# gabry1998/Self-Supervised-Anomaly-Detection

Hardware: AMD Instinct MI355X
Metric: train images/sec + anomaly-maps/sec, ResNet-18 256x256 bs256 (higher is better)
Workload: dtype f32; 1 GPU; ResNet-18 256x256 bs256 self-sup train + anomaly map, 1xMI355X, synthetic images (BASELINE configs[1]); images_per_gpu=256, global_batch=256, patches_per_image=841, bank_rows=588, parallelism=dp1 (256 images), train_step_launch=hipGraph segments, train_graph_segments=1

## Files before the change

### self-supervised-anomaly-detection_amd/csrc/stem.hip

```cpp
#include "common.h"
#include <type_traits>

namespace {

constexpr int STEM_MAX_GRID = 4096;


constexpr int TOH = 8, TOW = 32;
constexpr int TIH = TOH * 2 + 5;
constexpr int TIW = 72;
constexpr int KSTEPS = 7 * 4 * 3;
constexpr int IN_TILE = TIH * TIW * 3;
constexpr int W_TILE = KSTEPS * 2 * 64;

struct StemParams {
    const float* img;
    const float* wk;
    const float* scale;
    const float* shift;
    float* out;
    int B, H, W, pd, ps, Hv, Wv, Ho, Wo, relu;
    int prow, pcol;
    int ph, pw;
    int tiles_y, tiles_x;
    int64_t total_tiles;
    int64_t Nsamp;
    int hwnc;
    double* stats;
};

__global__ __launch_bounds__(256, 2) void stem_conv7x7_kernel(StemParams p) {
    extern __shared__ __attribute__((aligned(16))) float lds[];
    float* wl = lds;
    float* tin = lds + W_TILE;
    const int tid = threadIdx.x, lane = tid & 63, wave = tid >> 6;
    const int r = lane & 31, h = lane >> 5;

    for (int i = tid; i < W_TILE / 4; i += 256) ((f32x4*)wl)[i] = ((const f32x4*)p.wk)[i];

    float sc[2], sh[2];
#pragma unroll
    for (int j = 0; j < 2; ++j) {
        sc[j] = p.scale ? p.scale[j * 32 + r] : 1.f;
        sh[j] = p.shift ? p.shift[j * 32 + r] : 0.f;
    }

    double st0[2] = {0.0, 0.0}, st1[2] = {0.0, 0.0};
    const int tiles_per_sample = p.tiles_y * p.tiles_x;
    const bool direct = p.ph == p.Hv && p.pw == p.Wv;
    const int64_t plane = (int64_t)p.H * p.W;
    constexpr int NIN = (TIH * TIW + 255) / 256;
    float pv[NIN][3];
    auto fetch_tile = [&](int64_t t) {
        const int64_t n = t / tiles_per_sample;
        const int tt = (int)(t - n * tiles_per_sample);
        const int ty0 = (tt / p.tiles_x) * TOH, tx0 = (tt % p.tiles_x) * TOW;
        const int P = p.prow * p.pcol;
        const int b = (int)(n / P);
        const int pi = (int)(n - (int64_t)b * P);
        const int y0 = (pi / p.pcol) * p.ps, x0 = (pi % p.pcol) * p.ps;
        const float* src = p.img + (int64_t)b * 3 * plane;
#pragma unroll
        for (int q = 0; q < NIN; ++q) {
            const int i = tid + 256 * q;
            const int iy = i / TIW, ix = i - iy * TIW;
            const int vy = 2 * ty0 - 3 + iy, vx = 2 * tx0 - 3 + ix;
            float v0 = 0.f, v1 = 0.f, v2 = 0.f;
            if (i < TIH * TIW && (unsigned)vy < (unsigned)p.Hv && (unsigned)vx < (unsigned)p.Wv) {
                const int sy = y0 + (direct ? vy : (vy * p.ph) / p.Hv), sx = x0 + (direct ? vx : (vx * p.pw) / p.Wv);
                const float* s = src + (int64_t)sy * p.W + sx;
                v0 = s[0]; v1 = s[plane]; v2 = s[2 * plane];
            }
            pv[q][0] = v0; pv[q][1] = v1; pv[q][2] = v2;
        }
    };
    if ((int64_t)blockIdx.x < p.total_tiles) fetch_tile(blockIdx.x);
    for (int64_t t = blockIdx.x; t < p.total_tiles; t += gridDim.x) {
        const int64_t n = t / tiles_per_sample;
        const int tt = (int)(t - n * tiles_per_sample);
        const int ty0 = (tt / p.tiles_x) * TOH, tx0 = (tt % p.tiles_x) * TOW;

        __syncthreads();
#pragma unroll
        for (int q = 0; q < NIN; ++q) {
            const int i = tid + 256 * q;
            if (i < TIH * TIW) {
                float* d = tin + i * 3;
                d[0] = pv[q][0]; d[1] = pv[q][1]; d[2] = pv[q][2];
            }
        }
        __syncthreads();
        if (t + gridDim.x < p.total_tiles) fetch_tile(t + gridDim.x);

        f32x16 acc[2][2];
#pragma unroll
        for (int i = 0; i < 2; ++i)
#pragma unroll
            for (int j = 0; j < 2; ++j)
#pragma unroll
                for (int e = 0; e < 16; ++e) acc[i][j][e] = 0.f;
        const float* a0 = tin + ((2 * (2 * wave + 0)) * TIW + 2 * r + h) * 3;
        const float* a1 = tin + ((2 * (2 * wave + 1)) * TIW + 2 * r + h) * 3;
        const float* bw = wl + h * 64 + r;
#pragma unroll
        for (int ky = 0; ky < 7; ++ky)
#pragma unroll
            for (int q = 0; q < 4; ++q)
#pragma unroll
                for (int c = 0; c < 3; ++c) {
                    const int ko = (ky * TIW + 2 * q) * 3 + c;
                    const int kb = ((ky * 4 + q) * 3 + c) * 128;
                    float x0v = a0[ko], x1v = a1[ko];
                    float w0 = bw[kb], w1 = bw[kb + 32];
                    acc[0][0] = mfma32(x0v, w0, acc[0][0]);
                    acc[0][1] = mfma32(x0v, w1, acc[0][1]);
                    acc[1][0] = mfma32(x1v, w0, acc[1][0]);
                    acc[1][1] = mfma32(x1v, w1, acc[1][1]);
                }

        if (tx0 + 32 <= p.Wo) {
            const int64_t pst = p.hwnc ? p.Nsamp * 256 : 256;
            const unsigned lane_off = (unsigned)((int64_t)(4 * h) * pst + r * 4);
            typedef float f32x2v __attribute__((ext_vector_type(2)));
            auto rows = [&](auto stats_tag) __attribute__((always_inline)) {
                constexpr bool ST = decltype(stats_tag)::value;
                const float lowb = p.relu ? 0.f : -__builtin_huge_valf();
#pragma unroll
                for (int i = 0; i < 2; ++i) {
                    const int oy = ty0 + 2 * wave + i;
                    if (oy >= p.Ho) continue;
                    const int64_t pix0 = p.hwnc ? ((int64_t)oy * p.Wo + tx0) * p.Nsamp + n : (n * p.Ho + oy) * p.Wo + tx0;
                    char* const ob = (char*)(p.out + pix0 * 64);
#pragma unroll
                    for (int j = 0; j < 2; ++j) {
                        f32x2v ps = {0.f, 0.f}, pq = {0.f, 0.f};
#pragma unroll
                        for (int e = 0; e < 16; e += 2) {
                            f32x2v v = {acc[i][j][e], acc[i][j][e + 1]};
                            if (ST) {
                                ps += v;
                                pq = v * v + pq;
                            } else {
                                v = v * f32x2v{sc[j], sc[j]} + f32x2v{sh[j], sh[j]};
                                v[0] = fmaxf(v[0], lowb); v[1] = fmaxf(v[1], lowb);
                            }
#pragma unroll
                            for (int k = 0; k < 2; ++k)
                                *(float*)(ob + (int64_t)(((e + k) & 3) + 8 * ((e + k) >> 2)) * pst + j * 128 + lane_off) = v[k];
                        }
                        if (ST) { st0[j] += (double)ps[0] + (double)ps[1]; st1[j] += (double)pq[0] + (double)pq[1]; }
                    }
                }
            };
            if (p.stats && !p.scale && !p.shift && !p.relu) { rows(std::true_type()); continue; }
            if (!p.stats) { rows(std::false_type()); continue; }
        }
#pragma unroll
        for (int i = 0; i < 2; ++i) {
            const int oy = ty0 + 2 * wave + i;
            if (oy >= p.Ho) continue;
#pragma unroll
            for (int j = 0; j < 2; ++j) {
                float fs = 0.f, fq = 0.f;
#pragma unroll
                for (int e = 0; e < 16; ++e) {
                    int ox = tx0 + (e & 3) + 8 * (e >> 2) + 4 * h;
                    if (ox < p.Wo) {
                        if (p.stats) { fs += acc[i][j][e]; fq += acc[i][j][e] * acc[i][j][e]; }
                        float v = acc[i][j][e] * sc[j] + sh[j];
                        if (p.relu) v = fmaxf(v, 0.f);
                        const int64_t pix = p.hwnc ? ((int64_t)oy * p.Wo + ox) * p.Nsamp + n : (n * p.Ho + oy) * p.Wo + ox;
                        p.out[pix * 64 + j * 32 + r] = v;
                    }
                }
                if (p.stats) { st0[j] += (double)fs; st1[j] += (double)fq; }
            }
        }
    }
    if (p.stats) {
        __syncthreads();
        double* S = (double*)lds;
#pragma unroll
        for (int j = 0; j < 2; ++j) {
            st0[j] += __shfl_xor(st0[j], 32);
            st1[j] += __shfl_xor(st1[j], 32);
            if (h == 0) {
                S[(wave * 2 + 0) * 64 + j * 32 + r] = st0[j];
                S[(wave * 2 + 1) * 64 + j * 32 + r] = st1[j];
            }
        }
        __syncthreads();
        if (tid < 128) {
            const int which = tid >> 6, cc = tid & 63;
            p.stats[((int64_t)blockIdx.x * 2 + which) * 64 + cc] =
                ((S[(0 * 2 + which) * 64 + cc] + S[(1 * 2 + which) * 64 + cc]) + S[(2 * 2 + which) * 64 + cc]) + S[(3 * 2 + which) * 64 + cc];
        }
    }
}

constexpr int SP_SW = 40, SP_SH = 36;
constexpr int SP_SRC = SP_SH * SP_SW * 3;
constexpr int SP_WF = 24 * 2 * 64;
constexpr int SP_CB = 9 * 32 * 32;

struct StemPatchParams {
    const float* img;
    const float* wf;
    const float* scale;
    const float* shift;
    float* out;
    int B, H, W, ps, prow, pcol, hwnc;
    int skip_lo, skip_hi;
    int64_t Nsamp;
};

__global__ __launch_bounds__(256, 2) void stem_patch_fused_kernel(StemPatchParams p) {
    extern __shared__ __attribute__((aligned(16))) float lds[];
    float* wl = lds;
    float* src = lds + SP_WF;
    float* cb = src + SP_SRC;
    const int tid = threadIdx.x, lane = tid & 63, wave = tid >> 6;
    const int r = lane & 31, h = lane >> 5;
    for (int i = tid; i < SP_WF / 4; i += 256) ((f32x4*)wl)[i] = ((const f32x4*)p.wf)[i];
    const int P = p.prow * p.pcol;
    const int64_t plane = (int64_t)p.H * p.W;

    constexpr int NSRC = (SP_SH * SP_SW + 255) / 256;
    float pv[NSRC][3];
    auto fetch_patch = [&](int64_t n) {
        const int b = (int)(n / P);
        const int pi = (int)(n - (int64_t)b * P);
        const int y0 = (pi / p.pcol) * p.ps, x0 = (pi % p.pcol) * p.ps;
        const float* im = p.img + (int64_t)b * 3 * plane;
#pragma unroll
        for (int q = 0; q < NSRC; ++q) {
            const int i = tid + 256 * q;
            const int ty = i / SP_SW, tx = i - ty * SP_SW;
            const int sy = ty - 2, sx = tx - 2;
            float v0 = 0.f, v1 = 0.f, v2 = 0.f;
            if (i < SP_SH * SP_SW && (unsigned)sy < 32u && (unsigned)sx < 32u) {
                const float* s = im + (int64_t)(y0 + sy) * p.W + x0 + sx;
                v0 = s[0]; v1 = s[plane]; v2 = s[2 * plane];
            }
            pv[q][0] = v0; pv[q][1] = v1; pv[q][2] = v2;
        }
    };
    if ((int64_t)blockIdx.x < p.Nsamp) fetch_patch(blockIdx.x);
    for (int64_t n = blockIdx.x; n < p.Nsamp; n += gridDim.x) {
        __syncthreads();
#pragma unroll
        for (int q = 0; q < NSRC; ++q) {
            const int i = tid + 256 * q;
            if (i < SP_SH * SP_SW) {
                float* d = src + i * 3;
                d[0] = pv[q][0]; d[1] = pv[q][1]; d[2] = pv[q][2];
            }
        }
        if (n + gridDim.x < p.Nsamp) fetch_patch(n + gridDim.x);
        for (int pass = 0; pass < 2; ++pass) {
            const float sc = p.scale ? p.scale[pass * 32 + r] : 1.f;
            const float sh = p.shift ? p.shift[pass * 32 + r] : 0.f;
            for (int i = tid; i < 32 * 32; i += 256) cb[i] = 0.f;
            __syncthreads();
            for (int t = 0; t < 4; ++t) {
                f32x16 acc0, acc1;
#pragma unroll
                for (int e = 0; e < 16; ++e) { acc0[e] = 0.f; acc1[e] = 0.f; }
                const int oy = 8 * t + 2 * wave;
                const float* a0 = src + ((oy + 0) * SP_SW + r + h) * 3;
                const float* a1 = src + ((oy + 1) * SP_SW + r + h) * 3;
                const float* bw = wl + h * 64 + pass * 32 + r;
// ... 39 lines not shown
                ((f32x4*)cb)[tid] = ((const f32x4*)(cb + 8 * 32 * 32))[tid];
                __syncthreads();
            }
        }
    }
}

constexpr int SB_CB = 7 * 32 * 32;

__global__ __launch_bounds__(256, 2) void stem_patch_border_kernel(StemPatchParams p) {
    extern __shared__ __attribute__((aligned(16))) float lds[];
    float* wl = lds;
    float* src = lds + SP_WF;
    float* cb = src + SP_SRC;
    const int tid = threadIdx.x, lane = tid & 63, wave = tid >> 6;
    const int r = lane & 31, h = lane >> 5;
    for (int i = tid; i < SP_WF / 4; i += 256) ((f32x4*)wl)[i] = ((const f32x4*)p.wf)[i];
    const int P = p.prow * p.pcol;
    const int64_t plane = (int64_t)p.H * p.W;
    constexpr int NSRC = (SP_SH * SP_SW + 255) / 256;
    float pv[NSRC][3];
    auto fetch_patch = [&](int64_t n) {
        const int b = (int)(n / P);
        const int pi = (int)(n - (int64_t)b * P);
        const int y0 = (pi / p.pcol) * p.ps, x0 = (pi % p.pcol) * p.ps;
        const float* im = p.img + (int64_t)b * 3 * plane;
#pragma unroll
        for (int q = 0; q < NSRC; ++q) {
            const int i = tid + 256 * q;
            const int ty = i / SP_SW, tx = i - ty * SP_SW;
            const int sy = ty - 2, sx = tx - 2;
            float v0 = 0.f, v1 = 0.f, v2 = 0.f;
            if (i < SP_SH * SP_SW && (unsigned)sy < 32u && (unsigned)sx < 32u) {
                const float* s = im + (int64_t)(y0 + sy) * p.W + x0 + sx;
                v0 = s[0]; v1 = s[plane]; v2 = s[2 * plane];
            }
            pv[q][0] = v0; pv[q][1] = v1; pv[q][2] = v2;
        }
    };
    auto row_of = [](int t) { return t < 4 ? t : 25 + t; };
    const int ta0 = 2 * wave, ta1 = 2 * wave + 1 < 7 ? 2 * wave + 1 : 2 * wave;
    const float* pa0 = src + (row_of(ta0) * SP_SW + r + h) * 3;
    const float* pa1 = src + (row_of(ta1) * SP_SW + r + h) * 3;
    const float *pb0, *pb1;
    {
        int q0 = (2 * wave) * 32 + r, q1 = (2 * wave + 1) * 32 + r;
        q0 = q0 < 189 ? q0 : 188; q1 = q1 < 189 ? q1 : 188;
        const int c0 = q0 % 7, c1 = q1 % 7;
        pb0 = src + ((3 + q0 / 7) * SP_SW + (c0 < 4 ? c0 : 25 + c0) + h) * 3;
        pb1 = src + ((3 + q1 / 7) * SP_SW + (c1 < 4 ? c1 : 25 + c1) + h) * 3;
    }
    auto two_tiles = [&](const float* a0, const float* a1, int pass, f32x16& acc0, f32x16& acc1) {
#pragma unroll
        for (int e = 0; e < 16; ++e) { acc0[e] = 0.f; acc1[e] = 0.f; }
        const float* bw = wl + h * 64 + pass * 32 + r;
#pragma unroll
        for (int a = 0; a < 4; ++a)
#pragma unroll
            for (int q = 0; q < 2; ++q)
#pragma unroll
                for (int c = 0; c < 3; ++c) {
                    const int ko = (a * SP_SW + 2 * q) * 3 + c;
                    const float w = bw[((a * 2 + q) * 3 + c) * 128];
                    acc0 = mfma32(a0[ko], w, acc0);
                    acc1 = mfma32(a1[ko], w, acc1);
                }
    };
    if ((int64_t)blockIdx.x < p.Nsamp) fetch_patch(blockIdx.x);
    for (int64_t n = blockIdx.x; n < p.Nsamp; n += gridDim.x) {
        __syncthreads();
#pragma unroll
        for (int q = 0; q < NSRC; ++q) {
            const int i = tid + 256 * q;
            if (i < SP_SH * SP_SW) {
                float* d = src + i * 3;
                d[0] = pv[q][0]; d[1] = pv[q][1]; d[2] = pv[q][2];
            }
        }
        if (n + gridDim.x < p.Nsamp) fetch_patch(n + gridDim.x);
        __syncthreads();
        for (int pass = 0; pass < 2; ++pass) {
            const float sc = p.scale ? p.scale[pass * 32 + r] : 1.f;
            const float sh = p.shift ? p.shift[pass * 32 + r] : 0.f;
            f32x16 acc0, acc1;
            two_tiles(pa0, pa1, pass, acc0, acc1);
#pragma unroll
            for (int e = 0; e < 16; ++e) {
                const int ox = (e & 3) + 8 * (e >> 2) + 4 * h;
                cb[((2 * wave) * 32 + ox) * 32 + r] = fmaxf(acc0[e] * sc + sh, 0.f);
                if (2 * wave + 1 < 7) cb[((2 * wave + 1) * 32 + ox) * 32 + r] = fmaxf(acc1[e] * sc + sh, 0.f);
            }
            __syncthreads();
            for (int item = tid; item < 3 * 16 * 8; item += 256) {
                const int c4 = item & 7, px = (item >> 3) & 15, pr = item >> 7;
                const int t_lo = pr == 0 ? 0 : pr == 1 ? 1 : 4, t_hi = pr == 0 ? 1 : pr == 1 ? 3 : 6;
                f32x4 m = {0.f, 0.f, 0.f, 0.f};
                for (int t = t_lo; t <= t_hi; ++t)
#pragma unroll
                    for (int dx = -1; dx < 2; ++dx) {
                        const int cx = 2 * px + dx;
                        if (cx < 0) continue;
                        const f32x4 v = *(const f32x4*)(cb + (t * 32 + cx) * 32 + c4 * 4);
                        m[0] = fmaxf(m[0], v[0]); m[1] = fmaxf(m[1], v[1]); m[2] = fmaxf(m[2], v[2]); m[3] = fmaxf(m[3], v[3]);
                    }
                const int py = pr < 2 ? pr : 15;
                *(f32x4*)(p.out + (((int64_t)py * 16 + px) * p.Nsamp + n) * 64 + pass * 32 + c4 * 4) = m;
            }
            __syncthreads();
            if (wave < 3) {
                two_tiles(pb0, pb1, pass, acc0, acc1);
#pragma unroll
                for (int e = 0; e < 16; ++e) {
                    const int i = (e & 3) + 8 * (e >> 2) + 4 * h;
                    const int q0 = (2 * wave) * 32 + i, q1 = q0 + 32;
                    if (q0 < 189) cb[q0 * 32 + r] = fmaxf(acc0[e] * sc + sh, 0.f);
                    if (q1 < 189) cb[q1 * 32 + r] = fmaxf(acc1[e] * sc + sh, 0.f);
                }
            }
            __syncthreads();
            for (int item = tid; item < 13 * 3 * 8; item += 256) {
                const int c4 = item & 7, k = item >> 3, pk = k % 3, py = 2 + k / 3;
                const int ci_lo = pk == 0 ? 0 : pk == 1 ? 1 : 4, ci_hi = pk == 0 ? 1 : pk == 1 ? 3 : 6;
                f32x4 m = {0.f, 0.f, 0.f, 0.f};
#pragma unroll
                for (int dy = -1; dy < 2; ++dy)
                    for (int ci = ci_lo; ci <= ci_hi; ++ci) {
                        const f32x4 v = *(const f32x4*)(cb + ((2 * py + dy - 3) * 7 + ci) * 32 + c4 * 4);
                        m[0] = fmaxf(m[0], v[0]); m[1] = fmaxf(m[1], v[1]); m[2] = fmaxf(m[2], v[2]); m[3] = fmaxf(m[3], v[3]);
                    }
                const int px = pk < 2 ? pk : 15;
                *(f32x4*)(p.out + (((int64_t)py * 16 + px) * p.Nsamp + n) * 64 + pass * 32 + c4 * 4) = m;
            }
            __syncthreads();
        }
    }
}

__global__ void pack_stem_weight_folded_kernel(const float* __restrict__ w, float* __restrict__ wf) {
    const int i = blockIdx.x * blockDim.x + threadIdx.x;
    if (i >= SP_WF) return;
    const int co = i & 63, hh = (i >> 6) & 1, s = i >> 7;
    const int c = s % 3, q = (s / 3) & 1, a = s / 6;
    const int b = 2 * q + hh;
    const int ky0 = a == 0 ? 0 : 2 * a - 1, ky1 = a == 0 ? 0 : 2 * a;
    const int kx0 = b == 0 ? 0 : 2 * b - 1, kx1 = b == 0 ? 0 : 2 * b;
    float acc = 0.f;
    for (int ky = ky0; ky <= ky1; ++ky)
        for (int kx = kx0; kx <= kx1; ++kx) acc += w[((co * 3 + c) * 7 + ky) * 7 + kx];
    wf[i] = acc;
}

__global__ void pack_stem_weight_kernel(const float* __restrict__ w, float* __restrict__ wk, int ohwi = 0) {
    int i = blockIdx.x * blockDim.x + threadIdx.x;
    if (i >= 168 * 64) return;
    int co = i & 63, kl = i >> 6;
    int hh = kl & 1, rest = kl >> 1;
    int c = rest % 3, q = (rest / 3) & 3, ky = rest / 12;
    int kx = 2 * q + hh;
    const int src = ohwi ? ((co * 7 + ky) * 7 + (kx < 7 ? kx : 0)) * 3 + c : ((co * 3 + c) * 7 + ky) * 7 + (kx < 7 ? kx : 0);
    const float v = w[src];
    wk[i] = kx < 7 ? v : 0.f;
}

struct PoolBN { const float* mean; const float* invstd; const float* gamma; const float* beta; };

template <typename T>
__global__ __launch_bounds__(256) void maxpool3x3s2_kernel(const T* __restrict__ in, T* __restrict__ out, uint8_t* __restrict__ idx,
                                    int64_t totalE, int H, int W, int CE, int Ho, int Wo, int64_t N, int hwnc, PoolBN bn,
                                    T* __restrict__ zwin = nullptr) {
    constexpr int E = Lane<T>::E;
    using V = typename Lane<T>::vec;
    int64_t i = (int64_t)blockIdx.x * blockDim.x + threadIdx.x;
    if (i >= totalE) return;
    int cq = (int)(i % CE);
    int64_t pix = i / CE;
    int ox, oy;
    int64_t n;
    if (hwnc) {
        n = pix % N;
        int64_t t = pix / N;
        ox = (int)(t % Wo);
        oy = (int)(t / Wo);
    } else {
        ox = (int)(pix % Wo);
        int64_t t = pix / Wo;
        oy = (int)(t % Ho);
        n = t / Ho;
    }
    V m = -INFINITY, zw = 0.f;
    int am[E];
#pragma unroll
    for (int k = 0; k < E; ++k) am[k] = 0;
    V mu = 0.f, is = 0.f, ga = 0.f, be = 0.f;
    if (bn.mean) {
        mu = ldpar<V>(bn.mean, cq); is = ldpar<V>(bn.invstd, cq);
        ga = ldpar<V>(bn.gamma, cq); be = ldpar<V>(bn.beta, cq);
    }
    V tap[9];
#pragma unroll
    for (int dy = 0; dy < 3; ++dy) {
#pragma unroll
        for (int dx = 0; dx < 3; ++dx) {
            const int y = oy * 2 - 1 + dy, x = ox * 2 - 1 + dx;
            const bool ok = (unsigned)y < (unsigned)H && (unsigned)x < (unsigned)W;
            const int yc = ok ? y : oy * 2, xc = ok ? x : ox * 2;
            const int64_t ip = hwnc ? ((int64_t)yc * W + xc) * N + n : (n * H + yc) * W + xc;
            tap[dy * 3 + dx] = ldv(in + E * (ip * CE + cq));
        }
    }
#pragma unroll
    for (int dy = 0; dy < 3; ++dy) {
        int y = oy * 2 - 1 + dy;
        if ((unsigned)y >= (unsigned)H) continue;
#pragma unroll
        for (int dx = 0; dx < 3; ++dx) {
            int x = ox * 2 - 1 + dx;
            if ((unsigned)x >= (unsigned)W) continue;
            V v = tap[dy * 3 + dx];
            const V raw = v;
            if (bn.mean) {
#pragma unroll
                for (int k = 0; k < E; ++k) v[k] = stored<T>(fmaxf((v[k] - mu[k]) * is[k] * ga[k] + be[k], 0.f));
            }
#pragma unroll
            for (int k = 0; k < E; ++k)
                if (v[k] > m[k]) { m[k] = v[k]; am[k] = dy * 3 + dx; zw[k] = raw[k]; }
        }
    }
    stv(out + E * i, m);
    if (zwin) stv(zwin + E * i, zw);
    if (idx) {
#pragma unroll
        for (int q = 0; q < E / 4; ++q)
            ((uint32_t*)idx)[i * (E / 4) + q] = (uint32_t)am[4 * q] | ((uint32_t)am[4 * q + 1] << 8) | ((uint32_t)am[4 * q + 2] << 16) |
                                                ((uint32_t)am[4 * q + 3] << 24);
    }
}

}

extern "C" int ssad_pack_stem_weight(const float* w_oihw, float* wk, void* stream) {
    SSAD_CHECK_ARG(w_oihw && wk, "null pointer");
    hipLaunchKernelGGL(pack_stem_weight_kernel, dim3((168 * 64 + 255) / 256), dim3(256), 0, (hipStream_t)stream, w_oihw, wk, 0);
    SSAD_CHECK_LAUNCH();
    return 0;
}

extern "C" int ssad_pack_stem_weight_ohwi(const float* w_ohwi, float* wk, void* stream) {
    SSAD_CHECK_ARG(w_ohwi && wk, "null pointer");
    hipLaunchKernelGGL(pack_stem_weight_kernel, dim3((168 * 64 + 255) / 256), dim3(256), 0, (hipStream_t)stream, w_ohwi, wk, 1);
    SSAD_CHECK_LAUNCH();
    return 0;
}

static int stem_fwd_impl(const float* img, int B, int H, int W, int patch_dim, int patch_stride, int Hv, int Wv,
                         const float* wk, const float* scale, const float* shift, int relu, int hwnc, float* out,
                         void* stream, double* stats, int* stat_rows) {
    SSAD_CHECK_ARG(img && wk && out, "null pointer");
    SSAD_CHECK_ARG(B > 0 && H > 0 && W > 0 && Hv > 0 && Wv > 0, "empty shape");
    StemParams p;
    p.img = img; p.wk = wk; p.scale = scale; p.shift = shift; p.out = out;
    p.B = B; p.H = H; p.W = W; p.pd = patch_dim; p.ps = patch_stride; p.Hv = Hv; p.Wv = Wv; p.relu = relu;
    if (patch_dim > 0) {
        SSAD_CHECK_ARG(patch_stride > 0 && patch_dim <= H && patch_dim <= W, "bad patch window");
        p.prow = (H - patch_dim) / patch_stride + 1;
        p.pcol = (W - patch_dim) / patch_stride + 1;
        p.ph = p.pw = patch_dim;
    } else {
        p.prow = p.pcol = 1; p.ph = H; p.pw = W; p.ps = 0;
    }
    p.Ho = (Hv - 1) / 2 + 1;
    p.Wo = (Wv - 1) / 2 + 1;
    p.tiles_y = (p.Ho + TOH - 1) / TOH;
    p.tiles_x = (p.Wo + TOW - 1) / TOW;
    p.Nsamp = (int64_t)B * p.prow * p.pcol;
    p.hwnc = hwnc;
    p.stats = stats;
    p.total_tiles = p.Nsamp * p.tiles_y * p.tiles_x;
    constexpr int lds_bytes = (W_TILE + IN_TILE) * 4;
    static bool attr_set = false;
    if (!attr_set) {
        SSAD_SET_DYN_LDS(stem_conv7x7_kernel, lds_bytes);
        attr_set = true;
    }
    int64_t grid = p.total_tiles < STEM_MAX_GRID ? p.total_tiles : STEM_MAX_GRID;
    hipLaunchKernelGGL(stem_conv7x7_kernel, dim3((unsigned)grid), dim3(256), lds_bytes, (hipStream_t)stream, p);
    SSAD_CHECK_LAUNCH();
    if (stat_rows) *stat_rows = (int)grid;
    return 0;
}

extern "C" int ssad_stem_fwd(const float* img, int B, int H, int W, int patch_dim, int patch_stride, int Hv, int Wv,
                             const float* wk, const float* scale, const float* shift, int relu, int hwnc, float* out,
                             void* stream) {
    return stem_fwd_impl(img, B, H, W, patch_dim, patch_stride, Hv, Wv, wk, scale, shift, relu, hwnc, out, stream, nullptr, nullptr);
}

extern "C" int ssad_stem_stats_rows(void) { return STEM_MAX_GRID; }

extern "C" int ssad_stem_fwd_stats(const float* img, int B, int H, int W, int Hv, int Wv, const float* wk, float* out, float eps,
                                   float momentum, float* mean, float* invstd, float* running_mean, float* running_var,
                                   double* workspace, void* stream) {
    SSAD_CHECK_ARG(mean && invstd && workspace, "null pointer");
    int rows = 0;
    const int rc = stem_fwd_impl(img, B, H, W, 0, 0, Hv, Wv, wk, nullptr, nullptr, 0, 0, out, stream, workspace, &rows);
    if (rc) return rc;
    const int Ho = (Hv - 1) / 2 + 1, Wo = (Wv - 1) / 2 + 1;
    return ssad_bn_finalize_partials(workspace, rows, (int64_t)B * Ho * Wo, 64, eps, momentum, mean, invstd, running_mean,
                                     running_var, stream);
}

extern "C" int ssad_pack_stem_weight_folded(const float* w_oihw, float* wf, void* stream) {
    SSAD_CHECK_ARG(w_oihw && wf, "null pointer");
    hipLaunchKernelGGL(pack_stem_weight_folded_kernel, dim3((SP_WF + 255) / 256), dim3(256), 0, (hipStream_t)stream, w_oihw, wf);
    SSAD_CHECK_LAUNCH();
    return 0;
}

extern "C" int ssad_stem_patch_pool_fwd_ring(const float* img, int B, int H, int W, int patch_stride, const float* wf,
                                             const float* scale, const float* shift, int hwnc, int skip_lo, int skip_hi, float* out,
                                             void* stream);
extern "C" int ssad_stem_patch_pool_fwd(const float* img, int B, int H, int W, int patch_stride, const float* wf,
                                        const float* scale, const float* shift, int hwnc, float* out, void* stream) {
    return ssad_stem_patch_pool_fwd_ring(img, B, H, W, patch_stride, wf, scale, shift, hwnc, 1, 0, out, stream);
}
extern "C" int ssad_stem_patch_pool_fwd_ring(const float* img, int B, int H, int W, int patch_stride, const float* wf,
                                             const float* scale, const float* shift, int hwnc, int skip_lo, int skip_hi, float* out,
                                             void* stream) {
    SSAD_CHECK_ARG(img && wf && out, "null pointer");
    SSAD_CHECK_ARG(skip_lo > skip_hi || (skip_lo >= 0 && skip_hi < 16), "skipped square outside the 16 x 16 map");
    SSAD_CHECK_ARG(B > 0 && H >= 32 && W >= 32 && patch_stride > 0, "bad shape (32x32 windows)");
    StemPatchParams p;
    p.img = img; p.wf = wf; p.scale = scale; p.shift = shift; p.out = out;
    p.B = B; p.H = H; p.W = W; p.ps = patch_stride; p.hwnc = hwnc; p.skip_lo = skip_lo; p.skip_hi = skip_hi;
    p.prow = (H - 32) / patch_stride + 1;
    p.pcol = (W - 32) / patch_stride + 1;
    p.Nsamp = (int64_t)B * p.prow * p.pcol;
    constexpr int lds_bytes = (SP_WF + SP_SRC + SP_CB) * 4;
    static bool attr_set = false;
    if (!attr_set) {
        SSAD_SET_DYN_LDS(stem_patch_fused_kernel, lds_bytes);
        attr_set = true;
    }
    const int64_t grid = p.Nsamp < 2048 ? p.Nsamp : 2048;
    hipLaunchKernelGGL(stem_patch_fused_kernel, dim3((unsigned)grid), dim3(256), lds_bytes, (hipStream_t)stream, p);
    SSAD_CHECK_LAUNCH();
    return 0;
}

extern "C" int ssad_stem_patch_border_fwd(const float* img, int B, int H, int W, int patch_stride, const float* wf, const float* scale,
                                          const float* shift, float* out, void* stream) {
    SSAD_CHECK_ARG(img && wf && out, "null pointer");
    SSAD_CHECK_ARG(B > 0 && H >= 32 && W >= 32 && patch_stride > 0, "bad shape (32x32 windows)");
    StemPatchParams p;
    p.img = img; p.wf = wf; p.scale = scale; p.shift = shift; p.out = out;
    p.B = B; p.H = H; p.W = W; p.ps = patch_stride; p.hwnc = 1; p.skip_lo = 1; p.skip_hi = 0;
    p.prow = (H - 32) / patch_stride + 1;
    p.pcol = (W - 32) / patch_stride + 1;
    p.Nsamp = (int64_t)B * p.prow * p.pcol;
    constexpr int lds_bytes = (SP_WF + SP_SRC + SB_CB) * 4;
    static bool attr_set = false;
    if (!attr_set) {
        SSAD_SET_DYN_LDS(stem_patch_border_kernel, lds_bytes);
        attr_set = true;
    }
    const int64_t grid = p.Nsamp < 2048 ? p.Nsamp : 2048;
    hipLaunchKernelGGL(stem_patch_border_kernel, dim3((unsigned)grid), dim3(256), lds_bytes, (hipStream_t)stream, p);
    SSAD_CHECK_LAUNCH();
    return 0;
}

template <typename T>
static int maxpool_fwd_impl(const T* in, T* out, uint8_t* idx, int64_t N, int H, int W, int C, int hwnc, void* stream,
                            PoolBN bn = PoolBN{nullptr, nullptr, nullptr, nullptr}, T* zwin = nullptr) {
    SSAD_CHECK_ARG(in && out, "null pointer");
    SSAD_CHECK_ARG(N > 0 && H > 0 && W > 0 && C > 0 && C % 4 == 0, "bad shape (C % 4)");
    int Ho = (H - 1) / 2 + 1, Wo = (W - 1) / 2 + 1;
    constexpr int E = Lane<T>::E;
    SSAD_CHECK_ARG(C % E == 0, "channel count must be a multiple of the 16-byte lane width");
    int64_t totalE = N * Ho * Wo * (C / E);
    SSAD_CHECK_ARG(cdiv64(totalE, 256) < (int64_t)2147483647, "too large");
    hipLaunchKernelGGL(maxpool3x3s2_kernel<T>, dim3((unsigned)cdiv64(totalE, 256)), dim3(256), 0, (hipStream_t)stream, in, out, idx,
                       totalE, H, W, C / E, Ho, Wo, N, hwnc, bn, zwin);
    SSAD_CHECK_LAUNCH();
    return 0;
}

extern "C" int ssad_bn_relu_maxpool_fwd(const float* z, const float* mean, const float* invstd, const float* gamma,
                                        const float* beta, float* out, uint8_t* idx, int64_t N, int H, int W, int C,
                                        void* stream) {
    SSAD_CHECK_ARG(mean && invstd && gamma && beta && idx, "null pointer");
    return maxpool_fwd_impl<float>(z, out, idx, N, H, W, C, 0, stream, PoolBN{mean, invstd, gamma, beta});
}

extern "C" int ssad_bn_relu_maxpool_fwd_h(const void* z, const float* mean, const float* invstd, const float* gamma,
                                          const float* beta, void* out, uint8_t* idx, int64_t N, int H, int W, int C,
                                          void* stream) {
    SSAD_CHECK_ARG(mean && invstd && gamma && beta && idx, "null pointer");
    return maxpool_fwd_impl<hf>((const hf*)z, (hf*)out, idx, N, H, W, C, 0, stream, PoolBN{mean, invstd, gamma, beta});
}

extern "C" int ssad_bn_relu_maxpool_fwd_win(const float* z, const float* mean, const float* invstd, const float* gamma,
                                            const float* beta, float* out, uint8_t* idx, float* zwin, int64_t N, int H, int W, int C,
                                            void* stream) {
    SSAD_CHECK_ARG(mean && invstd && gamma && beta && idx && zwin, "null pointer");
    return maxpool_fwd_impl<float>(z, out, idx, N, H, W, C, 0, stream, PoolBN{mean, invstd, gamma, beta}, zwin);
}
extern "C" int ssad_bn_relu_maxpool_fwd_win_h(const void* z, const float* mean, const float* invstd, const float* gamma,
                                              const float* beta, void* out, uint8_t* idx, void* zwin, int64_t N, int H, int W, int C,
                                              void* stream) {
    SSAD_CHECK_ARG(mean && invstd && gamma && beta && idx && zwin, "null pointer");
    return maxpool_fwd_impl<hf>((const hf*)z, (hf*)out, idx, N, H, W, C, 0, stream, PoolBN{mean, invstd, gamma, beta}, (hf*)zwin);
}

extern "C" int ssad_maxpool3x3s2_fwd(const float* in, float* out, int64_t N, int H, int W, int C, int hwnc, void* stream) {
    return maxpool_fwd_impl<float>(in, out, nullptr, N, H, W, C, hwnc, stream);
}

extern "C" int ssad_maxpool3x3s2_fwd_idx(const float* in, float* out, uint8_t* idx, int64_t N, int H, int W, int C, void* stream) {
    SSAD_CHECK_ARG(idx, "null index buffer");
    return maxpool_fwd_impl<float>(in, out, idx, N, H, W, C, 0, stream);
}
```

### self-supervised-anomaly-detection_amd/self_supervised/ops.py

```python
import os

import torch

from . import _hip


PROFILE = None


def _new(shape, like):
    return torch.empty(shape, device=like.device, dtype=torch.float32)


def _newh(shape, like):
    return torch.empty(shape, device=like.device, dtype=torch.float16)


def _is_h(t):
    return t is not None and t.dtype == torch.float16


def _p(t, allow_none=False):
    return _hip.ptr(t, allow_none, torch.float16 if _is_h(t) else torch.float32)


def _run(kernel, flops, nbytes, rc_fn, exec_flops=None, tile=None):
    if PROFILE is None:
        _hip.check(rc_fn())
        return
    e0, e1 = torch.cuda.Event(enable_timing=True), torch.cuda.Event(enable_timing=True)
    e0.record()
    _hip.check(rc_fn())
    e1.record()
    PROFILE.append((kernel, flops, nbytes, e0, e1, flops if exec_flops is None else exec_flops, tile() if tile else None))


ASIDE = None


def _run_aside(kernel, flops, nbytes, rc_fn, keep=()):
    if ASIDE is None or PROFILE is not None:
        return _run(kernel, flops, nbytes, rc_fn)
    ASIDE.launch(lambda: _hip.check(rc_fn()), keep)


PENDING_REDUCE = None


def _wgrad_reduce(slab, dw_out, splits, cout, kpad, kh, kw, cin, to_oihw, accumulate):
    kreal = kh * kw * cin
    if (PENDING_REDUCE is not None and PROFILE is None and not to_oihw and not accumulate and kreal % 4 == 0 and kpad % 4 == 0
            and slab.data_ptr() % 16 == 0 and dw_out.data_ptr() % 16 == 0):
        PENDING_REDUCE.append((slab, dw_out, int(splits), int(cout), int(kpad), int(kreal)))
        return
    _run_aside("wgrad_reduce", 0.0, 4.0 * slab.numel(),
               lambda: _hip.lib().ssad_wgrad_reduce(_hip.ptr(slab), _hip.ptr(dw_out), splits, cout, kpad, kh, kw, cin, int(to_oihw),
                                                    int(accumulate), _hip.stream()), keep=(slab,))


def flush_reductions():
    if not PENDING_REDUCE:
        return
    import ctypes
    desc = []
    for slab, out, splits, cout, kpad, kreal in PENDING_REDUCE:
        desc += [slab.data_ptr(), out.data_ptr(), splits, cout, kpad, kreal]
    arr = (ctypes.c_int64 * len(desc))(*desc)
    _hip.check(_hip.lib().ssad_wgrad_reduce_batch(arr, len(PENDING_REDUCE), _hip.stream()))
    del PENDING_REDUCE[:]


def drain_profile():
    global PROFILE
    recs = PROFILE or []
    torch.cuda.synchronize()
    out = [{"kernel": k, "flops": f, "bytes": b, "ms": e0.elapsed_time(e1), "exec_flops": x, "tile": t}
           for k, f, b, e0, e1, x, t in recs]
    PROFILE = [] if PROFILE is not None else None
    return out


def _inbounds_taps(h, w, kh, kw, stride, pad):
    ho, wo = (h + 2 * pad - kh) // stride + 1, (w + 2 * pad - kw) // stride + 1
    ny = sum(sum(1 for ky in range(kh) if 0 <= oy * stride - pad + ky < h) for oy in range(ho))
    nx = sum(sum(1 for kx in range(kw) if 0 <= ox * stride - pad + kx < w) for ox in range(wo))
    return ny * nx


IGEMM_FWD, IGEMM_HWNC, IGEMM_RING, IGEMM_STATS, IGEMM_DGRAD = range(5)


IGEMM_TILES = [("256x64_K16", (256, 64, 2, 2, 16, True)), ("256x64_SB", (256, 64, 2, 2, 32, False)),
               ("128x64", (128, 64, 1, 2, 32, True)), ("256x128", (256, 128, 2, 2, 32, True)),
               ("256x128_W4", (256, 128, 4, 2, 32, True)), ("128x256", (128, 256, 2, 4, 32, True)),
               ("64x64", (64, 64, 1, 1, 32, True)), ("128x128", (128, 128, 2, 2, 32, True)),
               ("256x256", (256, 256, 4, 4, 32, True)), ("128x64_SB", (128, 64, 1, 2, 32, False)),
               ("128x64_K16", (128, 64, 1, 2, 16, True)), ("128x128_K16", (128, 128, 2, 2, 16, True)),
               ("128x256_K16", (128, 256, 2, 4, 16, True))]
LINEAR_SMALL = "linear_small"


def igemm_tile(n, h, w, cin, cout, kh, kw, stride, pad, mode):
    k = cout if mode == IGEMM_DGRAD else cin
    if (mode in (IGEMM_FWD, IGEMM_STATS, IGEMM_DGRAD) and kh == kw == h == w == 1 and stride == 1 and pad == 0 and k % 4 == 0
            and n <= _hip.lib().ssad_linear_small_max_rows()):
        return LINEAR_SMALL, False
    t = _hip.lib().ssad_conv_igemm_tile_id(n, h, w, cin, cout, kh, kw, stride, pad, int(mode))
    return IGEMM_TILES[t % 100][0], t >= 100


def igemm_tile_name(n, h, w, cin, cout, kh, kw, stride, pad, mode):
    name, pos = igemm_tile(n, h, w, cin, cout, kh, kw, stride, pad, mode)
    if name == LINEAR_SMALL:
        return "<linear_small: 32 x 32 tiles, csrc/linear_small.hip>"
    bm, bn, tm, tn, bk, db = dict(IGEMM_TILES)[name]
    ts = stride if mode == IGEMM_DGRAD else 1
    return f"<{bm},{bn},{tm},{tn},{bk},{ts},{'true' if pos else 'false'}{'' if db else ',false'}>"


def _kname(base, mode):
    return base + {0: "_f32", 1: "_bf16", 2: "_f16", 3: "_x3", 6: "_x6"}[int(mode)]


def repack_oihw_to_ohwi(w):
    o, i, kh, kw = w.shape
    out = _new((o, kh, kw, i), w)
    _hip.check(_hip.lib().ssad_repack_oihw_to_ohwi(_hip.ptr(w), _hip.ptr(out), o, i, kh, kw, _hip.stream()))
    return out


def repack_ohwi_to_oihw(w):
    o, kh, kw, i = w.shape
    out = _new((o, i, kh, kw), w)
    _hip.check(_hip.lib().ssad_repack_ohwi_to_oihw(_hip.ptr(w), _hip.ptr(out), o, i, kh, kw, _hip.stream()))
    return out


def pack_stem_weight(w):
    out = _new((168, 64), w)
    if tuple(w.shape) == (64, 7, 7, 3):
        _hip.check(_hip.lib().ssad_pack_stem_weight_ohwi(_hip.ptr(w), _hip.ptr(out), _hip.stream()))
        return out
    assert tuple(w.shape) == (64, 3, 7, 7)
    _hip.check(_hip.lib().ssad_pack_stem_weight(_hip.ptr(w), _hip.ptr(out), _hip.stream()))
    return out


def stem_geometry(H, W, patch_dim, patch_stride):
    if patch_dim:
        p = ((H - patch_dim) // patch_stride + 1) * ((W - patch_dim) // patch_stride + 1)
        wh = ww = patch_dim
    else:
        p, wh, ww = 1, H, W
    hv, wv = (64, 64) if (wh < 64 or ww < 64) else (wh, ww)
    return p, hv, wv, (hv - 1) // 2 + 1, (wv - 1) // 2 + 1


def stem_fwd(img, wk, scale, shift, relu=True, patch_dim=0, patch_stride=0, hwnc=False, resize_to=None):
    b, c, h, w = img.shape
    assert c == 3
    p, hv, wv, ho, wo = stem_geometry(h, w, patch_dim, patch_stride)
    if resize_to is not None:
        assert not patch_dim
        hv, wv = resize_to
        ho, wo = (hv - 1) // 2 + 1, (wv - 1) // 2 + 1
    n = b * p
    out = _new((ho, wo, n, 64) if hwnc else (n, ho, wo, 64), img)
    _run("stem_conv7x7", 2.0 * n * ho * wo * 64 * 147, 4.0 * (b * 3 * h * w + n * ho * wo * 64),
         lambda: _hip.lib().ssad_stem_fwd(_hip.ptr(img), b, h, w, patch_dim, patch_stride, hv, wv, _hip.ptr(wk),
                                          _hip.ptr(scale, True), _hip.ptr(shift, True), int(relu), int(hwnc),
                                          _hip.ptr(out), _hip.stream()))
    return out


def stem_fwd_stats(img, wk, eps, momentum, running_mean, running_var):
    b, c, h, w = img.shape
    assert c == 3
    _, hv, wv, ho, wo = stem_geometry(h, w, 0, 0)
    out = _new((b, ho, wo, 64), img)
    mean, invstd = _new((64,), img), _new((64,), img)
    ws = torch.empty(_hip.lib().ssad_stem_stats_rows() * 128, device=img.device, dtype=torch.float64)
    _run("stem_conv7x7", 2.0 * b * ho * wo * 64 * 147, 4.0 * (b * 3 * h * w + b * ho * wo * 64),
         lambda: _hip.lib().ssad_stem_fwd_stats(_hip.ptr(img), b, h, w, hv, wv, _hip.ptr(wk), _hip.ptr(out), eps, momentum,
                                                _hip.ptr(mean), _hip.ptr(invstd), _hip.ptr(running_mean, True),
                                                _hip.ptr(running_var, True), ws.data_ptr(), _hip.stream()))
    return out, mean, invstd


def stem_fwd_stats16(img, w_oihw, eps, momentum, running_mean, running_var, mode, out_half=False):
    b, c, h, w = img.shape
    ohwi = tuple(w_oihw.shape) == (64, 7, 7, 3)
    assert c == 3 and (ohwi or tuple(w_oihw.shape) == (64, 3, 7, 7)) and int(mode) in (1, 2)
    assert h >= 64 and w >= 64, "images below 64 x 64 are resized first (models.py:217-219): that is the fp32 stem's loader"
    lib = _hip.lib()
    wk = torch.empty(14 * 64 * 16, device=img.device, dtype=torch.float16 if int(mode) == 2 else torch.bfloat16)
    _hip.check((lib.ssad_pack_stem_weight16_ohwi if ohwi else lib.ssad_pack_stem_weight16)(_hip.ptr(w_oihw), wk.data_ptr(), int(int(mode) == 2),
                                                                                             _hip.stream()))
    ho, wo = (h - 1) // 2 + 1, (w - 1) // 2 + 1
    mean, invstd = _new((64,), img), _new((64,), img)
    ws = torch.empty(lib.ssad_stem_stats_rows() * 128, device=img.device, dtype=torch.float64)
    if out_half:
        assert int(mode) == 2
        out = _newh((b, ho, wo, 64), img)
        _run("stem_conv7x7_h16", 2.0 * b * ho * wo * 64 * 147, 4.0 * b * 3 * h * w + 2.0 * b * ho * wo * 64,
             lambda: lib.ssad_stem_fwd_stats16_h(_hip.ptr(img), b, h, w, wk.data_ptr(), out.data_ptr(), eps, momentum, _hip.ptr(mean),
                                                 _hip.ptr(invstd), _hip.ptr(running_mean, True), _hip.ptr(running_var, True),
                                                 ws.data_ptr(), _hip.stream()))
        return out, mean, invstd
    out = _new((b, ho, wo, 64), img)
    _run(_kname("stem_conv7x7", mode), 2.0 * b * ho * wo * 64 * 147, 4.0 * (b * 3 * h * w + b * ho * wo * 64),
         lambda: lib.ssad_stem_fwd_stats16(_hip.ptr(img), b, h, w, wk.data_ptr(), _hip.ptr(out), eps, momentum, _hip.ptr(mean),
                                           _hip.ptr(invstd), _hip.ptr(running_mean, True), _hip.ptr(running_var, True),
                                           ws.data_ptr(), int(int(mode) == 2), _hip.stream()))
    return out, mean, invstd


def pack_stem_weight_folded(w):
    assert tuple(w.shape) == (64, 3, 7, 7)
    out = _new((24, 2, 64), w)
    _hip.check(_hip.lib().ssad_pack_stem_weight_folded(_hip.ptr(w), _hip.ptr(out), _hip.stream()))
    return out


def stem_patch_pool_fwd(img, wf, scale, shift, patch_stride=8, hwnc=False, skip=None):
    b, c, h, w = img.shape
    n = b * ((h - 32) // patch_stride + 1) * ((w - 32) // patch_stride + 1)
    out = _new((16, 16, n, 64) if hwnc else (n, 16, 16, 64), img)
    lo, hi = skip if skip is not None else (1, 0)
    _run("stem_patch_pool", 2.0 * n * 32 * 32 * 64 * 147, 4.0 * (img.numel() + out.numel()),
         lambda: _hip.lib().ssad_stem_patch_pool_fwd_ring(_hip.ptr(img), b, h, w, patch_stride, _hip.ptr(wf), _hip.ptr(scale, True),
                                                          _hip.ptr(shift, True), int(hwnc), lo, hi, _hip.ptr(out), _hip.stream()))
    return out


def stem_patch_border_fwd(img, wf, scale, shift, patch_stride=8):
    b, c, h, w = img.shape
    n = b * ((h - 32) // patch_stride + 1) * ((w - 32) // patch_stride + 1)
    out = _new((16, 16, n, 64), img)
    _run("stem_patch_pool", 2.0 * n * 13 * 32 * 64 * 147, 4.0 * (img.numel() + out.numel() * 87 // 256),
         lambda: _hip.lib().ssad_stem_patch_border_fwd(_hip.ptr(img), b, h, w, patch_stride, _hip.ptr(wf), _hip.ptr(scale, True),
                                                       _hip.ptr(shift, True), _hip.ptr(out), _hip.stream()))
    return out


def maxpool3x3s2_fwd(x, hwnc=False):
    if hwnc:
        h, w, n, c = x.shape
        out = _new(((h - 1) // 2 + 1, (w - 1) // 2 + 1, n, c), x)
    else:
        n, h, w, c = x.shape
        out = _new((n, (h - 1) // 2 + 1, (w - 1) // 2 + 1, c), x)
    _run("maxpool3x3s2", 0.0, 4.0 * (x.numel() + out.numel()),
         lambda: _hip.lib().ssad_maxpool3x3s2_fwd(_hip.ptr(x), _hip.ptr(out), n, h, w, c, int(hwnc), _hip.stream()))
    return out


def _split_fwd(mode):
    return _hip.lib().ssad_conv_igemm_fwd_x6 if mode == 6 else _hip.lib().ssad_conv_igemm_fwd_x3


def conv_fwd_hwnc(x, w_ohwi, scale=None, shift=None, residual=None, relu=False, stride=1, pad=0, x3=False):
    h, w, n, cin = x.shape
    cout, kh, kw, cin2 = w_ohwi.shape
    assert cin == cin2
    ho, wo = (h + 2 * pad - kh) // stride + 1, (w + 2 * pad - kw) // stride + 1
    out = _new((ho, wo, n, cout), x)
    nb = 4.0 * (x.numel() + out.numel() * (2 if residual is not None else 1) + w_ohwi.numel())
    if x3:
        _run("conv_igemm_x6" if x3 == 6 else "conv_igemm_x3", 2.0 * out.numel() * kh * kw * cin, nb,
             lambda: _split_fwd(x3)(_hip.ptr(x), _hip.ptr(w_ohwi), _hip.ptr(out), _hip.ptr(scale, True),
                                    _hip.ptr(shift, True), _hip.ptr(residual, True), int(relu), n, h, w,
                                    cin, cout, kh, kw, stride, pad, 1, _hip.stream()))
        return out
    _run("conv_igemm_pos_f32", 2.0 * out.numel() * kh * kw * cin, nb,
         lambda: _hip.lib().ssad_conv_igemm_fwd_hwnc(_hip.ptr(x), _hip.ptr(w_ohwi), _hip.ptr(out), _hip.ptr(scale, True),
                                                     _hip.ptr(shift, True), _hip.ptr(residual, True), int(relu), n, h, w,
                                                     cin, cout, kh, kw, stride, pad, _hip.stream()),
         exec_flops=2.0 * n * cout * cin * _inbounds_taps(h, w, kh, kw, stride, pad) if PROFILE is not None else None,
         tile=lambda: igemm_tile_name(n, h, w, cin, cout, kh, kw, stride, pad, IGEMM_HWNC))
    return out


def conv_fwd_hwnc_ring(x, w_ohwi, scale, shift, residual, relu, skip_lo, skip_hi):
    h, w, n, cin = x.shape
    cout, kh, kw, cin2 = w_ohwi.shape
    assert cin == cin2 and (kh, kw) == (3, 3) and 0 <= skip_lo <= skip_hi < min(h, w)
    out = _new((h, w, n, cout), x)
    side = skip_hi - skip_lo + 1
    ring = h * w - side * side
    taps = _inbounds_taps(h, w, 3, 3, 1, 1) - 9 * side * side if PROFILE is not None else 0
    _run("conv_igemm_pos_f32", 2.0 * n * ring * cout * 9 * cin, 4.0 * (x.numel() + n * ring * cout * (2 if residual is not None else 1) + w_ohwi.numel()),
         lambda: _hip.lib().ssad_conv_igemm_fwd_hwnc_ring(_hip.ptr(x), _hip.ptr(w_ohwi), _hip.ptr(out), _hip.ptr(scale, True),
# ... 1655 lines not shown
```

Measured before the change: 8222 images/sec.

## Double-buffer stem input tile in LDS and trim padded K steps

```diff
diff --git a/self-supervised-anomaly-detection_amd/csrc/stem.hip b/self-supervised-anomaly-detection_amd/csrc/stem.hip
--- a/self-supervised-anomaly-detection_amd/csrc/stem.hip
+++ b/self-supervised-anomaly-detection_amd/csrc/stem.hip
@@ -1,4 +1,5 @@
 #include "common.h"
+#include <stdlib.h>
 #include <type_traits>
 
 namespace {
@@ -9,7 +10,8 @@
 constexpr int TOH = 8, TOW = 32;
 constexpr int TIH = TOH * 2 + 5;
 constexpr int TIW = 72;
-constexpr int KSTEPS = 7 * 4 * 3;
+constexpr int KROW = 22;
+constexpr int KSTEPS = 7 * KROW / 2;
 constexpr int IN_TILE = TIH * TIW * 3;
 constexpr int W_TILE = KSTEPS * 2 * 64;
 
@@ -74,23 +76,31 @@
             pv[q][0] = v0; pv[q][1] = v1; pv[q][2] = v2;
         }
     };
-    if ((int64_t)blockIdx.x < p.total_tiles) fetch_tile(blockIdx.x);
+    auto store_tile = [&](float* dst) {
+#pragma unroll
+        for (int q = 0; q < NIN; ++q) {
+            const int i = tid + 256 * q;
+            if (i < TIH * TIW) {
+                float* d = dst + i * 3;
+                d[0] = pv[q][0]; d[1] = pv[q][1]; d[2] = pv[q][2];
+            }
+        }
+    };
+    if ((int64_t)blockIdx.x < p.total_tiles) {
+        fetch_tile(blockIdx.x);
+        store_tile(tin);
+        if ((int64_t)blockIdx.x + gridDim.x < p.total_tiles) fetch_tile((int64_t)blockIdx.x + gridDim.x);
+    }
+    int buf = 0;
     for (int64_t t = blockIdx.x; t < p.total_tiles; t += gridDim.x) {
         const int64_t n = t / tiles_per_sample;
         const int tt = (int)(t - n * tiles_per_sample);
         const int ty0 = (tt / p.tiles_x) * TOH, tx0 = (tt % p.tiles_x) * TOW;
+        const float* cur = tin + buf * IN_TILE;
+        float* nxt = tin + (buf ^ 1) * IN_TILE;
+        buf ^= 1;
 
         __syncthreads();
-#pragma unroll
-        for (int q = 0; q < NIN; ++q) {
-            const int i = tid + 256 * q;
-            if (i < TIH * TIW) {
-                float* d = tin + i * 3;
-                d[0] = pv[q][0]; d[1] = pv[q][1]; d[2] = pv[q][2];
-            }
-        }
-        __syncthreads();
-        if (t + gridDim.x < p.total_tiles) fetch_tile(t + gridDim.x);
 
         f32x16 acc[2][2];
 #pragma unroll
@@ -99,24 +109,31 @@
             for (int j = 0; j < 2; ++j)
 #pragma unroll
                 for (int e = 0; e < 16; ++e) acc[i][j][e] = 0.f;
-        const float* a0 = tin + ((2 * (2 * wave + 0)) * TIW + 2 * r + h) * 3;
-        const float* a1 = tin + ((2 * (2 * wave + 1)) * TIW + 2 * r + h) * 3;
-        const float* bw = wl + h * 64 + r;
-#pragma unroll
-        for (int ky = 0; ky < 7; ++ky)
-#pragma unroll
-            for (int q = 0; q < 4; ++q)
-#pragma unroll
-                for (int c = 0; c < 3; ++c) {
-                    const int ko = (ky * TIW + 2 * q) * 3 + c;
-                    const int kb = ((ky * 4 + q) * 3 + c) * 128;
-                    float x0v = a0[ko], x1v = a1[ko];
-                    float w0 = bw[kb], w1 = bw[kb + 32];
+        const float* ab0 = cur + ((2 * (2 * wave + 0)) * TIW + 2 * r) * 3;
+        const float* ab1 = cur + ((2 * (2 * wave + 1)) * TIW + 2 * r) * 3;
+        const float *a0[2] = {ab0 + 3 * h, ab0 + h}, *a1[2] = {ab1 + 3 * h, ab1 + h};
+        const float* bw[2] = {wl + 3 * h * 64 + r, wl + h * 64 + r};
+        auto filter_rows = [&](auto ky_lo, auto ky_hi) __attribute__((always_inline)) {
+#pragma unroll
+            for (int ky = decltype(ky_lo)::value; ky < decltype(ky_hi)::value; ++ky)
+#pragma unroll
+                for (int s = 0; s < KROW / 2; ++s) {
+                    const int u = s < 9 ? 0 : 1;
+                    const int j = s < 9 ? 6 * (s / 3) + s % 3 : 18 + 2 * (s - 9);
+                    const int ko = ky * TIW * 3 + j;
+                    const int kb = (ky * KROW + j) * 64;
+                    float x0v = a0[u][ko], x1v = a1[u][ko];
+                    float w0 = bw[u][kb], w1 = bw[u][kb + 32];
                     acc[0][0] = mfma32(x0v, w0, acc[0][0]);
                     acc[0][1] = mfma32(x0v, w1, acc[0][1]);
                     acc[1][0] = mfma32(x1v, w0, acc[1][0]);
                     acc[1][1] = mfma32(x1v, w1, acc[1][1]);
                 }
+        };
+        filter_rows(std::integral_constant<int, 0>(), std::integral_constant<int, 3>());
+        if (t + gridDim.x < p.total_tiles) store_tile(nxt);
+        if (t + 2 * (int64_t)gridDim.x < p.total_tiles) fetch_tile(t + 2 * (int64_t)gridDim.x);
+        filter_rows(std::integral_constant<int, 3>(), std::integral_constant<int, 7>());
 
         if (tx0 + 32 <= p.Wo) {
             const int64_t pst = p.hwnc ? p.Nsamp * 256 : 256;
@@ -462,14 +479,12 @@
 
 __global__ void pack_stem_weight_kernel(const float* __restrict__ w, float* __restrict__ wk, int ohwi = 0) {
     int i = blockIdx.x * blockDim.x + threadIdx.x;
-    if (i >= 168 * 64) return;
+    if (i >= W_TILE) return;
     int co = i & 63, kl = i >> 6;
-    int hh = kl & 1, rest = kl >> 1;
-    int c = rest % 3, q = (rest / 3) & 3, ky = rest / 12;
-    int kx = 2 * q + hh;
-    const int src = ohwi ? ((co * 7 + ky) * 7 + (kx < 7 ? kx : 0)) * 3 + c : ((co * 3 + c) * 7 + ky) * 7 + (kx < 7 ? kx : 0);
-    const float v = w[src];
-    wk[i] = kx < 7 ? v : 0.f;
+    int ky = kl / KROW, j = kl - ky * KROW;
+    int kx = j / 3, c = j - kx * 3;
+    if (kx == 7) { wk[i] = 0.f; return; }
+    wk[i] = w[ohwi ? ((co * 7 + ky) * 7 + kx) * 3 + c : ((co * 3 + c) * 7 + ky) * 7 + kx];
 }
 
 struct PoolBN { const float* mean; const float* invstd; const float* gamma; const float* beta; };
@@ -551,14 +566,14 @@
 
 extern "C" int ssad_pack_stem_weight(const float* w_oihw, float* wk, void* stream) {
     SSAD_CHECK_ARG(w_oihw && wk, "null pointer");
-    hipLaunchKernelGGL(pack_stem_weight_kernel, dim3((168 * 64 + 255) / 256), dim3(256), 0, (hipStream_t)stream, w_oihw, wk, 0);
+    hipLaunchKernelGGL(pack_stem_weight_kernel, dim3((W_TILE + 255) / 256), dim3(256), 0, (hipStream_t)stream, w_oihw, wk, 0);
     SSAD_CHECK_LAUNCH();
     return 0;
 }
 
 extern "C" int ssad_pack_stem_weight_ohwi(const float* w_ohwi, float* wk, void* stream) {
     SSAD_CHECK_ARG(w_ohwi && wk, "null pointer");
-    hipLaunchKernelGGL(pack_stem_weight_kernel, dim3((168 * 64 + 255) / 256), dim3(256), 0, (hipStream_t)stream, w_ohwi, wk, 1);
+    hipLaunchKernelGGL(pack_stem_weight_kernel, dim3((W_TILE + 255) / 256), dim3(256), 0, (hipStream_t)stream, w_ohwi, wk, 1);
     SSAD_CHECK_LAUNCH();
     return 0;
 }
@@ -587,13 +602,17 @@
     p.hwnc = hwnc;
     p.stats = stats;
     p.total_tiles = p.Nsamp * p.tiles_y * p.tiles_x;
-    constexpr int lds_bytes = (W_TILE + IN_TILE) * 4;
+    constexpr int lds_bytes = (W_TILE + 2 * IN_TILE) * 4;
     static bool attr_set = false;
     if (!attr_set) {
         SSAD_SET_DYN_LDS(stem_conv7x7_kernel, lds_bytes);
         attr_set = true;
     }
     int64_t grid = p.total_tiles < STEM_MAX_GRID ? p.total_tiles : STEM_MAX_GRID;
+    if (const char* cap = getenv("SSAD_STEM_BLOCKS")) {
+        const int c = atoi(cap);
+        if (c > 0 && c < grid) grid = c;
+    }
     hipLaunchKernelGGL(stem_conv7x7_kernel, dim3((unsigned)grid), dim3(256), lds_bytes, (hipStream_t)stream, p);
     SSAD_CHECK_LAUNCH();
     if (stat_rows) *stat_rows = (int)grid;
diff --git a/self-supervised-anomaly-detection_amd/self_supervised/ops.py b/self-supervised-anomaly-detection_amd/self_supervised/ops.py
--- a/self-supervised-anomaly-detection_amd/self_supervised/ops.py
+++ b/self-supervised-anomaly-detection_amd/self_supervised/ops.py
@@ -137,7 +137,7 @@
 
 
 def pack_stem_weight(w):
-    out = _new((168, 64), w)
+    out = _new((154, 64), w)
     if tuple(w.shape) == (64, 7, 7, 3):
         _hip.check(_hip.lib().ssad_pack_stem_weight_ohwi(_hip.ptr(w), _hip.ptr(out), _hip.stream()))
         return out
```

After: 8208 images/sec. No clear change (-0.2%).
